# flo-audio/flo

Hardware: AMD Instinct MI355X
Metric: Msamples/s encoded (44.1k stereo, q=high) (higher is better)
Workload: dtype f32

## Files before the change

### diag/lds_model.py

```python
#!/usr/bin/env python3
import argparse
import re
from collections import Counter

import numpy as np

N, HOP, NB = 2048, 1024, 25
SLOT_CAP = 96
ROW = 1024
EDGES = np.array([0, 100, 200, 300, 400, 510, 630, 770, 920, 1080, 1270, 1480, 1720, 2000, 2320, 2700, 3150, 3700,
                  4400, 5300, 6400, 7700, 9500, 12000, 15500, 20500], dtype=np.float32)

R_WIN, R_TW, R_F1, R_F2, R_LANE, R_KEEP, R_DST, R_S10 = 0, 8, 12, 16, 20, 21, 25, 32


def bands(rate):
    res = np.float32(rate) / np.float32(N)
    band = []
    for k in range(HOP):
        f = (np.float32(k) + np.float32(0.5)) * res
        b = NB - 1
        for i in range(1, 26):
            if f < EDGES[i]:
                b = i - 1
# ... 24 lines not shown
    return lane_bnd, lane_slot0, band_slot0, dirty


G128 = [[0, 1, 2, 3, 12, 13, 14, 15] + list(range(20, 28)), [4, 5, 6, 7, 8, 9, 10, 11, 16, 17, 18, 19] + list(range(28, 32))]
G128 = G128 + [[l + 32 for l in g] for g in G128]
G32 = [list(range(0, 32)), list(range(32, 64))]


def contig(n):
    return [list(range(i, i + n)) for i in range(0, 64, n)]


RULES = {
    "ds_read_b32": [(G32, 1, 32)], "ds_write_b32": [(G32, 1, 32)], "ds_write_b16": [(G32, 1, 32)],
    "ds_read_b64": [(G32, 2, 64)], "ds_read_b128": [(G128, 4, 64)],
    "ds_read2_b32": [(G32, 1, 32), (G32, 1, 32)], "ds_write2_b32": [(G32, 1, 32), (G32, 1, 32)],
    "ds_read2_b64": [(contig(16), 2, 32), (contig(16), 2, 32)],
    "ds_write_b64": [(contig(16), 2, 32)], "ds_write_b128": [(contig(8), 4, 32)],
    "ds_write2_b64": [(contig(16), 2, 32), (contig(16), 2, 32)],
}
SKIP_EMPTY = False
GATHER_MASKS = False


def cost(kind, addrs):
    acc = RULES[kind]
    lists = addrs if len(acc) == 2 else [addrs]
    cyc = base = 0
    for (groups, dw, nbank), ad in zip(acc, lists):
        for g in groups:
            per_bank = {}
            for l in g:
                if ad[l] is None:
                    continue
                for i in range(dw):
                    d = ad[l] // 4 + i
                    per_bank.setdefault(d % nbank, set()).add(d)
            if SKIP_EMPTY and not per_bank:
                continue
            cyc += max([len(v) for v in per_bank.values()] or [1])
            base += 1
    return cyc, cyc - base


def lanes(f):
    return [f(l) for l in range(64)]


def sites(rate, layout):
    lane_bnd, lane_slot0, band_slot0, dirty = band_tables(rate)
    row = lambda r, off=0: lanes(lambda l: r * ROW + 16 * l + off)
    uni = lambda a: lanes(lambda l: a)
    one = lambda a: [a] + [None] * 63
    S = []
    S += [("frame", "peek consumed / coef counters", "ds_read_b32", uni(0x8000))] * 2
    S += [("frame", "kRowS10 (uniform)", "ds_read_b128", uni(R_S10 * ROW))] * 2
    if layout == "old":
        S += [("frame", "rcount: kRowLane .z", "ds_read_b32", row(R_LANE, 8))]
    else:
        S += [("frame", "rcount: kRowS10 dword 64 + lane", "ds_read_b32", lanes(lambda l: R_S10 * ROW + 256 + 4 * l))]
    for ph, rr in (("fft pass 1", R_F1), ("fft pass 2", R_F2)):
        S += [(ph, "twiddle rows", "ds_read_b128", row(rr + k)) for k in range(3)]
        S += [(ph, "twiddle row 4 (.xy)", "ds_read_b64", row(rr + 3))]
    X = 0x10000
    for ka in range(8):
        S += [("fft exchange 1", "writes", "ds_write_b128", lanes(lambda l: X + 16 * ((8 * ka + (l & 7)) * 9 + (l >> 3))))]
    for r in range(8):
        S += [("fft exchange 1", "reads", "ds_read_b128", lanes(lambda l: X + 16 * (l * 9 + r)))]
    T = X + 16000
    S += [("masking pass", "ts_ready peek", "ds_read_b32", uni(0x8004))]
    S += [("masking pass", "ts (tl, sf)", "ds_write2_b32", [lanes(lambda l: T + 16 * (l & 31) + 4 * (l >> 5) + o if (l & 31) < 25 else None) for o in (0, 8)])]
    S += [("masking pass", "sfwh", "ds_write_b16", lanes(lambda l: T + 1024 + 2 * l if (l & 31) < 25 else None))]
    S += [("masking pass", "alive", "ds_write_b64", one(T + 1200))]
    S += [("masking pass", "ts_ready", "ds_write_b32", one(0x8004))]
    for kb in range(8):
        S += [("fft exchange 2", "writes", "ds_write_b128", lanes(lambda l: X + 16 * (((l >> 3) + 8 * kb) * 9 + (l & 7))))]
    for r in range(8):
        S += [("fft exchange 2", "reads", "ds_read_b128", lanes(lambda l: X + 16 * (l * 9 + r)))]
    pl = lambda l: 2 * l + 2 * (l >> 3)
    for r in range(8):
        if layout == "old" or r % 2 == 0:
            if layout == "old":
                S += [("post-rotation", "twiddle rows (half rows)", "ds_read_b64", row(R_TW + r // 2, 8 * (r & 1)))]
            else:
                S += [("post-rotation", "twiddle rows", "ds_read_b128", row(R_TW + r // 2))]
        S += [("post-rotation", "transpose writes (2m)", "ds_write_b64", lanes(lambda l: X + 8 * (pl(l) + 144 * r)))]
        S += [("post-rotation", "transpose writes (1023-2m)", "ds_write_b64", lanes(lambda l: X + 8 * (1149 - pl(l) - 144 * r)))]
    for q in range(8):
        S += [("post-rotation", "transpose reads", "ds_read_b128", lanes(lambda l: X + 16 * (9 * l) + 16 * q))]
    S += [("band statistics", "coef_ready", "ds_write_b32", one(0x8008))]
    es = [e for e in range(16) if (dirty >> e) & 1]
    if layout == "old":
        for rr in (R_KEEP, R_DST):
            for g in range(4):
                comp = [e - 4 * g for e in es if 4 * g <= e < 4 * g + 4 and (rr == R_DST or e < 15)]
                i = 0
                while i < len(comp):
                    if i + 1 < len(comp) and comp[i + 1] == comp[i] + 1 and comp[i] % 2 == 1:
                        S += [("band statistics", "keep / dst rows (dword pieces)", "ds_read2_b32", [row(rr + g, 4 * comp[i]), row(rr + g, 4 * comp[i] + 4)])]
                        i += 2
                    elif i + 1 < len(comp) and comp[i + 1] == comp[i] + 1:
                        S += [("band statistics", "keep / dst rows (dword pieces)", "ds_read_b64", row(rr + g, 4 * comp[i]))]
                        i += 2
                    else:
                        S += [("band statistics", "keep / dst rows (dword pieces)", "ds_read_b32", row(rr + g, 4 * comp[i]))]
                        i += 1
    elif layout == "new":
        S += [("band statistics", "keep / dst rows (whole rows)", "ds_read_b128", row(rr + g)) for rr in (R_KEEP, R_DST) for g in range(4)]
    SL = X + 9216
    masks = layout == "masks"
    for e in es:
        def dst(l, e=e, off=0):
            m = lane_bnd[l]
            if (m >> e) & 1:
                return SL + 16 * (lane_slot0[l] + bin(m & ((1 << e) - 1)).count("1")) + off
            return None if masks else SL + 16 * (SLOT_CAP + l)
        if masks and e == 15:
            S += [("band statistics", "slot store (element 15, all lanes)", "ds_write_b128", lanes(dst))]
        elif masks:
            S += [("band statistics", "slot stores (closing lanes)", "ds_write2_b64", [lanes(dst), lanes(lambda l: dst(l, off=8))])]
        else:
            S += [("band statistics", "slot stores", "ds_write_b128", lanes(dst))]
    zero = SLOT_CAP + 64
    for u in range(12):
        def src(l, u=u):
            b = min(l & 31, 24)
            bs0 = band_slot0[b] + (l >> 5)
            bs1 = band_slot0[b + 1] if (l & 31) < 25 else 0
            s = bs0 + 2 * u
            if masks and GATHER_MASKS and not bs0 + 2 * 4 * (u // 4) < bs1:
                return None
            return SL + 16 * (s if s < bs1 else zero)
        S += [("band statistics", "slot gathers", "ds_read_b128", lanes(src))]
    for r in range(8):
        S += [("fold", "window rows", "ds_read_b128", row(R_WIN + r))]
    if layout == "old":
        for k in range(4):
            S += [("fold", "twiddle rows (read2_b64)", "ds_read2_b64", [row(R_TW + k), row(R_TW + k, 8)])]
    else:
        S += [("fold", "twiddle rows", "ds_read_b128", row(R_TW + k)) for k in range(4)]
    return S


def isa_mix(path):
    txt = open(path).read().split("\n")
    start = next(i for i, t in enumerate(txt) if re.match(r"^_ZN3flo20lossy_chain2q_kernelILb0ELj(\d+)ELb0EE.*:", t)
                 and "Lj65535E" not in t)
    body = txt[start:]
    e = next(i for i, t in enumerate(body) if re.match(r"^\.LBB\d+_\d+:.*_clEjS\d_S\d_S\d_S\d_\.exit", t))
    a = max(i for i, t in enumerate(body[:e]) if re.match(r"^\.LBB\d+_\d+:\s+; %\.lr\.ph\d*$", t))
    lab = body[e].split(":")[0]
    c = next(i for i, t in enumerate(body) if i > a and re.search(r"s_cbranch\w*\s+" + re.escape(lab) + r"\b", t))
    b = next(i for i, t in enumerate(body) if i > e and re.match(r"^\.LBB", t))
    mix, cold = Counter(), Counter()
    for i in range(a, b):
        m = re.search(r"\b(ds_[a-z0-9_]+)", body[i])
        if m:
            (cold if c <= i < e else mix)[m.group(1)] += 1
    return mix, cold


def main():
    ap = argparse.ArgumentParser()
    ap.add_argument("--rate", type=int, default=44100)
    ap.add_argument("--layout", default="old", choices=["old", "new", "masks"])
    ap.add_argument("--skip-empty", action="store_true")
    ap.add_argument("--gather-masks", action="store_true")
    ap.add_argument("--isa")
    a = ap.parse_args()
    global SKIP_EMPTY, GATHER_MASKS
    SKIP_EMPTY, GATHER_MASKS = a.skip_empty, a.gather_masks
    S = sites(a.rate, a.layout)
    tab = {}
    tot_c = tot_x = 0
    for ph, site, kind, ad in S:
        c, x = cost(kind, ad)
        k = (ph, site, kind)
        n, cc, xx = tab.get(k, (0, 0, 0))
        tab[k] = (n + 1, cc + c, xx + x)
        tot_c += c
        tot_x += x
    print(f"{'phase':16} {'site':38} {'instruction':14} {'n':>3} {'array':>6} {'conflict':>8}")
    for (ph, site, kind), (n, c, x) in tab.items():
        print(f"{ph:16} {site:38} {kind:14} {n:3d} {c:6d} {x:8d}")
    print(f"{'transform wave, one stereo frame':70} {len(S):3d} {tot_c:6d} {tot_x:8d}")
    if a.isa:
        mix, cold = isa_mix(a.isa)
        model = Counter(kind for _, _, kind, _ in S)
        print("ISA mix (one frame):", dict(sorted(mix.items())), " cold loop (not run at this rate):", dict(cold))
        print("model mix          :", dict(sorted(model.items())))


if __name__ == "__main__":
    main()
```

### flo_amd/csrc/lossy_device.hpp

```cpp
#pragma once
#include <hip/hip_runtime.h>
#include <stdint.h>

#include "pack_rows.h"

namespace flo {


struct LossyDevTables {
    const float4 *pack;
    const float4 *pack_g;
    const float4 *pack_ext;
    const float *ath_db;
    const uint8_t *band;
    const float *band_count;
    const float *s10d;
    const uint32_t *lane_bnd;
    const uint32_t *lane_slot0;
    const uint32_t *band_slot0;
    int max_band_slots;
    uint32_t dirty;
    float smr_thr;
    int q_transparent;
};
// ... 278 lines not shown
    const char *base = reinterpret_cast<const char *>(pcm + s0 * nch + c0);
    const unsigned stride = 4u * (unsigned)nch;
#pragma unroll
    for (int r = 0; r < 8; r++) {
        int eo, oo;
        half_offsets(lane, r, eo, oo);
        const unsigned be = (unsigned)eo * stride, bo = (unsigned)oo * stride;
        if (CH == 2) {
            float2 a = *reinterpret_cast<const float2 *>(base + be);
            float2 b = *reinterpret_cast<const float2 *>(base + bo);
            he[0][r] = a.x;
            he[CH - 1][r] = a.y;
            ho[0][r] = b.x;
            ho[CH - 1][r] = b.y;
        } else {
            he[0][r] = *reinterpret_cast<const float *>(base + be);
            ho[0][r] = *reinterpret_cast<const float *>(base + bo);
        }
    }
}

template <int CH>
__device__ __forceinline__ void fold(const int lane, const float (&ae)[CH][8], const float (&ao)[CH][8], const float (&be)[CH][8],
                                     const float (&bo)[CH][8], float (&zr)[CH][8], float (&zi)[CH][8],
                                     const LossyDevTables &T) {
#pragma unroll
    for (int r = 0; r < 8; r++) {
        const float4 ww = T.pack[(kRowWin + r) * 64 + lane];
        const float wae = ww.x, wao = ww.y, wbe = ww.z, wbo = ww.w;
        const float4 t4 = T.pack[(kRowTw + (r >> 1)) * 64 + lane];
        const float2 w = (r & 1) ? make_float2(t4.z, t4.w) : make_float2(t4.x, t4.y);
#pragma unroll
        for (int c = 0; c < CH; c++) {
            float re, im;
            if (r < 4) {
                re = fmaf(-bo[c][r], wbo, -(be[c][r] * wbe));
                im = fmaf(ao[c][r], wao, -(ae[c][r] * wae));
            } else {
                re = fmaf(-ao[c][r], wao, ae[c][r] * wae);
                im = fmaf(-bo[c][r], wbo, -(be[c][r] * wbe));
            }
            zr[c][r] = fmaf(-im, w.y, -(re * w.x));
            zi[c][r] = fmaf(re, w.y, -(im * w.x));
        }
    }
}

template <int CH>
__device__ __forceinline__ void post_rotate_transpose(const int lane, const float (&zr)[CH][8], const float (&zi)[CH][8],
                                                      float (*coef)[kCoefFloats], float (&c)[CH][16],
                                                      const LossyDevTables &T) {
#pragma unroll
    for (int r = 0; r < 8; r++) {
        const int m = lane + 64 * r;
        const float4 t4 = T.pack[(kRowTw + (r >> 1)) * 64 + lane];
        const float2 w = (r & 1) ? make_float2(t4.z, t4.w) : make_float2(t4.x, t4.y);
        const int k0 = 2 * m, k1 = 1023 - 2 * m;
        const int p0 = k0 + 4 * (k0 >> 5), p1 = k1 + 4 * (k1 >> 5);
#pragma unroll
        for (int ch = 0; ch < CH; ch++) {
            float R = fmaf(-zi[ch][r], w.y, -(zr[ch][r] * w.x));
            float I = fmaf(zi[ch][r], w.x, -(zr[ch][r] * w.y));
            coef[ch][p0] = R;
            coef[ch][p1] = I;
        }
    }
    wave_sync();
#pragma unroll
    for (int ch = 0; ch < CH; ch++) {
        const float4 *p = reinterpret_cast<const float4 *>(&coef[ch][16 * lane + 4 * (lane >> 1)]);
#pragma unroll
        for (int q = 0; q < 4; q++) {
            float4 v = p[q];
            c[ch][4 * q + 0] = v.x;
            c[ch][4 * q + 1] = v.y;
            c[ch][4 * q + 2] = v.z;
            c[ch][4 * q + 3] = v.w;
        }
    }
    wave_sync();
}

typedef float v2f __attribute__((ext_vector_type(2)));
__device__ __forceinline__ v2f fma2(v2f a, v2f b, v2f c) { return __builtin_elementwise_fma(a, b, c); }
__device__ __forceinline__ v2f fma2_na_hi_nc(v2f a, v2f w, v2f c) {
    v2f r;
    asm("v_pk_fma_f32 %0, %1, %2, %3 op_sel:[0,1,0] op_sel_hi:[1,1,1] neg_lo:[1,0,1] neg_hi:[1,0,1]" : "=v"(r) : "v"(a), "v"(w), "v"(c));
    return r;
}
__device__ __forceinline__ v2f fma2_a_hi_c(v2f a, v2f w, v2f c) {
    v2f r;
    asm("v_pk_fma_f32 %0, %1, %2, %3 op_sel:[0,1,0] op_sel_hi:[1,1,1]" : "=v"(r) : "v"(a), "v"(w), "v"(c));
    return r;
}
__device__ __forceinline__ v2f mul2_hi(v2f a, v2f w) {
    v2f r;
    asm("v_pk_mul_f32 %0, %1, %2 op_sel:[0,1] op_sel_hi:[1,1]" : "=v"(r) : "v"(a), "v"(w));
    return r;
}
__device__ __forceinline__ v2f fma2_a_hi_nc(v2f a, v2f w, v2f c) {
    v2f r;
    asm("v_pk_fma_f32 %0, %1, %2, %3 op_sel:[0,1,0] op_sel_hi:[1,1,1] neg_lo:[0,0,1] neg_hi:[0,0,1]" : "=v"(r) : "v"(a), "v"(w), "v"(c));
    return r;
}
__device__ __forceinline__ v2f splat2(float x) { return (v2f){x, x}; }

constexpr int kXch4 = 64 * kXchStride;
constexpr int kCoef2 = 1024 + 2 * 64;

__device__ __forceinline__ void dft8_2(v2f *xr, v2f *xi) {
    const v2f s = splat2(0.70710678118654752440f);
    v2f a0r = xr[0] + xr[4], a0i = xi[0] + xi[4];
    v2f a1r = xr[0] - xr[4], a1i = xi[0] - xi[4];
    v2f a2r = xr[2] + xr[6], a2i = xi[2] + xi[6];
    v2f a3r = xr[2] - xr[6], a3i = xi[2] - xi[6];
    v2f a4r = xr[1] + xr[5], a4i = xi[1] + xi[5];
    v2f a5r = xr[1] - xr[5], a5i = xi[1] - xi[5];
    v2f a6r = xr[3] + xr[7], a6i = xi[3] + xi[7];
    v2f a7r = xr[3] - xr[7], a7i = xi[3] - xi[7];
    v2f b0r = a0r + a2r, b0i = a0i + a2i;
    v2f b2r = a0r - a2r, b2i = a0i - a2i;
    v2f b1r = a1r + a3i, b1i = a1i - a3r;
    v2f b3r = a1r - a3i, b3i = a1i + a3r;
    v2f c0r = a4r + a6r, c0i = a4i + a6i;
    v2f c2r = a4r - a6r, c2i = a4i - a6i;
    v2f c1r = a5r + a7i, c1i = a5i - a7r;
    v2f c3r = a5r - a7i, c3i = a5i + a7r;
    const v2f e1r = c1r + c1i, e1i = c1i - c1r;
    const v2f e3r = c3i - c3r, e3i = c3r + c3i;
    xr[0] = b0r + c0r; xi[0] = b0i + c0i;
    xr[4] = b0r - c0r; xi[4] = b0i - c0i;
    xr[1] = fma2(e1r, s, b1r); xi[1] = fma2(e1i, s, b1i);
    xr[5] = fma2(-e1r, s, b1r); xi[5] = fma2(-e1i, s, b1i);
    xr[2] = b2r + c2i; xi[2] = b2i - c2r;
    xr[6] = b2r - c2i; xi[6] = b2i + c2r;
    xr[3] = fma2(e3r, s, b3r); xi[3] = fma2(-e3i, s, b3i);
    xr[7] = fma2(-e3r, s, b3r); xi[7] = fma2(e3i, s, b3i);
}

__device__ __forceinline__ void cmul_2(v2f &xr, v2f &xi, float wr, float wi) {
    const v2f WR = splat2(wr), WI = splat2(wi);
    v2f r = fma2(xr, WR, -(xi * WI));
    v2f i = fma2(xr, WI, xi * WR);
    xr = r;
    xi = i;
}
__device__ __forceinline__ void cmul_2_pair(v2f &xr, v2f &xi, v2f w) {
    const v2f WR = splat2(w.x);
    v2f r = fma2(xr, WR, -mul2_hi(xi, w));
    v2f i = fma2_a_hi_c(xr, w, xi * WR);
    xr = r;
    xi = i;
}

struct NoShadow { __device__ __forceinline__ void operator()() const {} };
template <typename F = NoShadow>
__device__ __forceinline__ void fft512_2(const int lane, v2f (&zr)[8], v2f (&zi)[8], float4 *x4, const LossyDevTables &T, F &&shadow = F()) {
    dft8_2(zr, zi);
#pragma unroll
    for (int kk = 0; kk < 4; kk++) {
        const float4 w = T.pack[(kRowF1 + kk) * 64 + lane];
        cmul_2(zr[2 * kk + 1], zi[2 * kk + 1], w.x, w.y);
        if (kk < 3) cmul_2_pair(zr[2 * kk + 2], zi[2 * kk + 2], (v2f){w.z, w.w});
    }
    {
        const int nb = lane >> 3, nc = lane & 7;
#pragma unroll
        for (int ka = 0; ka < 8; ka++) x4[(8 * ka + nc) * kXchStride + nb] = make_float4(zr[ka].x, zr[ka].y, zi[ka].x, zi[ka].y);
        wave_sync();
#pragma unroll
        for (int r = 0; r < 8; r++) {
            const float4 v = x4[lane * kXchStride + r];
            zr[r] = (v2f){v.x, v.y};
            zi[r] = (v2f){v.z, v.w};
        }
        shadow();
        wave_sync();
    }
    dft8_2(zr, zi);
#pragma unroll
    for (int kk = 0; kk < 4; kk++) {
        const float4 w = T.pack[(kRowF2 + kk) * 64 + lane];
        cmul_2(zr[2 * kk + 1], zi[2 * kk + 1], w.x, w.y);
        if (kk < 3) cmul_2_pair(zr[2 * kk + 2], zi[2 * kk + 2], (v2f){w.z, w.w});
    }
    {
        const int ka = lane >> 3, nc = lane & 7;
#pragma unroll
        for (int kb = 0; kb < 8; kb++) x4[(ka + 8 * kb) * kXchStride + nc] = make_float4(zr[kb].x, zr[kb].y, zi[kb].x, zi[kb].y);
        wave_sync();
#pragma unroll
        for (int r = 0; r < 8; r++) {
            const float4 v = x4[lane * kXchStride + r];
            zr[r] = (v2f){v.x, v.y};
            zi[r] = (v2f){v.z, v.w};
        }
        wave_sync();
    }
    dft8_2(zr, zi);
}

__device__ __forceinline__ void load_half_fast_2(const int lane, const float *__restrict__ pcm, long long s0, v2f (&he)[8], v2f (&ho)[8]) {
    const char *base0 = reinterpret_cast<const char *>(pcm + s0 * 2);
    const char *base1 = base0 + 4096;
    const unsigned va = 16u * (unsigned)lane, vb = 16u * (unsigned)(63 - lane);
#pragma unroll
    for (int r = 0; r < 8; r++) {
        const int rr = r & 3;
        const char *pe = (r < 4 ? base1 : base0) + va + 1024 * rr;
        const char *po = (r < 4 ? base0 : base1) + vb + (3080 - 1024 * rr);
        const float2 a = *reinterpret_cast<const float2 *>(pe);
        const float2 b = *reinterpret_cast<const float2 *>(po);
        he[r] = (v2f){a.x, a.y};
        ho[r] = (v2f){b.x, b.y};
    }
}

__device__ __forceinline__ void fold_2(const int lane, const v2f (&ae)[8], const v2f (&ao)[8], const v2f (&be)[8], const v2f (&bo)[8],
                                       v2f (&zr)[8], v2f (&zi)[8], const LossyDevTables &T) {
    float4 t4;
#pragma unroll
    for (int r = 0; r < 8; r++) {
        const float4 ww = T.pack[(kRowWin + r) * 64 + lane];
        const v2f wae = splat2(ww.x), wao = splat2(ww.y), wbe = splat2(ww.z);
        const v2f whi = {ww.z, ww.w};
        if (!(r & 1)) t4 = pack_row(&T.pack[(kRowTw + (r >> 1)) * 64 + lane]);
        const v2f wx = splat2((r & 1) ? t4.z : t4.x);
        const v2f thi = {t4.z, t4.w};
        v2f re, im;
        if (r < 4) {
            re = fma2_na_hi_nc(bo[r], whi, be[r] * wbe);
            im = fma2(ao[r], wao, -(ae[r] * wae));
        } else {
            re = fma2(-ao[r], wao, ae[r] * wae);
            im = fma2_na_hi_nc(bo[r], whi, be[r] * wbe);
        }
        if (r & 1) {
            zr[r] = fma2_na_hi_nc(im, thi, re * wx);
            zi[r] = fma2_a_hi_nc(re, thi, im * wx);
        } else {
            const v2f wy = splat2(t4.y);
            zr[r] = fma2(-im, wy, -(re * wx));
            zi[r] = fma2(re, wy, -(im * wx));
        }
    }
}

__device__ __forceinline__ void post_rotate_transpose_2(const int lane, const v2f (&zr)[8], const v2f (&zi)[8], float2 *c2,
                                                        v2f (&c)[16], const LossyDevTables &T) {
    const int pl = 2 * lane + 2 * (lane >> 3);
    float2 *const w0 = c2 + pl;
    float2 *const w1 = c2 + (1149 - 7 * 144) - pl;
    float4 t4;
#pragma unroll
    for (int r = 0; r < 8; r++) {
        if (!(r & 1)) t4 = pack_row(&T.pack[(kRowTw + (r >> 1)) * 64 + lane]);
        const v2f wx = splat2((r & 1) ? t4.z : t4.x);
        v2f R, I;
        if (r & 1) {
            const v2f thi = {t4.z, t4.w};
            R = fma2_na_hi_nc(zi[r], thi, zr[r] * wx);
            I = fma2(zi[r], wx, -mul2_hi(zr[r], thi));
        } else {
            const v2f wy = splat2(t4.y);
            R = fma2(-zi[r], wy, -(zr[r] * wx));
            I = fma2(zi[r], wx, -(zr[r] * wy));
        }
        w0[144 * r] = make_float2(R.x, R.y);
        w1[144 * (7 - r)] = make_float2(I.x, I.y);
    }
    wave_sync();
    const float4 *p = reinterpret_cast<const float4 *>(&c2[18 * lane]);
#pragma unroll
    for (int q = 0; q < 8; q++) {
        const float4 v = p[q];
        c[2 * q] = (v2f){v.x, v.y};
        c[2 * q + 1] = (v2f){v.z, v.w};
    }
    wave_sync();
}

struct LaneConst {
    float rcount;
};

__device__ __forceinline__ void load_lane_const(const int lane, LaneConst &L, const LossyDevTables &T) {
    L.rcount = T.pack[kRowLane * 64 + lane].z;
}

constexpr int kZeroSlot = kSlotCap + 64;

template <int CH>
__device__ __forceinline__ void band_stats(const int lane, const float (&c)[CH][16], float2 (*slots)[kSlotCap + 64 + 1],
                                           const LossyDevTables &T, float (&energy)[CH], float (&bmax)[CH]) {
    float kp[16];
    uint32_t dv[16], so[12];
#pragma unroll
    for (int g = 0; g < 4; g++) {
        const float4 keep = T.pack[(kRowKeep + g) * 64 + lane];
        const float4 dsto = T.pack[(kRowDst + g) * 64 + lane];
        kp[4 * g + 0] = keep.x, kp[4 * g + 1] = keep.y, kp[4 * g + 2] = keep.z, kp[4 * g + 3] = keep.w;
        dv[4 * g + 0] = __float_as_uint(dsto.x), dv[4 * g + 1] = __float_as_uint(dsto.y);
        dv[4 * g + 2] = __float_as_uint(dsto.z), dv[4 * g + 3] = __float_as_uint(dsto.w);
    }
#pragma unroll
    for (int g = 0; g < 3; g++) {
        const float4 lst = T.pack[(kRowLst + g) * 64 + lane];
        so[4 * g + 0] = __float_as_uint(lst.x), so[4 * g + 1] = __float_as_uint(lst.y);
        so[4 * g + 2] = __float_as_uint(lst.z), so[4 * g + 3] = __float_as_uint(lst.w);
    }
    __builtin_amdgcn_sched_barrier(0);
    float acc[CH], mx[CH];
#pragma unroll
    for (int ch = 0; ch < CH; ch++) {
        acc[ch] = 0.f;
        mx[ch] = 0.f;
    }
#pragma unroll
    for (int e = 0; e < 16; e++) {
#pragma unroll
        for (int ch = 0; ch < CH; ch++) {
            acc[ch] = fmaf(c[ch][e], c[ch][e], acc[ch]);
            mx[ch] = max_abs_raw(mx[ch], c[ch][e]);
            *reinterpret_cast<float2 *>(reinterpret_cast<char *>(slots[ch]) + dv[e]) = make_float2(acc[ch], mx[ch]);
            acc[ch] *= kp[e];
            mx[ch] *= kp[e];
        }
    }
    wave_sync();
    float2 v[CH][12];
#pragma unroll
    for (int u = 0; u < 12; u++)
#pragma unroll
        for (int ch = 0; ch < CH; ch++)
            v[ch][u] = *reinterpret_cast<const float2 *>(reinterpret_cast<const char *>(slots[ch]) + so[u]);
    __builtin_amdgcn_sched_barrier(0);
#pragma unroll
    for (int ch = 0; ch < CH; ch++) {
        energy[ch] = 0.f;
        bmax[ch] = 0.f;
    }
#pragma unroll
    for (int u = 0; u < 12; u++)
#pragma unroll
        for (int ch = 0; ch < CH; ch++) {
            energy[ch] += v[ch][u].x;
            bmax[ch] = max_raw(bmax[ch], v[ch][u].y);
        }
    const int groups = (T.max_band_slots + 7) >> 3;
    for (int g = 3; g < groups; g++) {
// ... 916 lines not shown
```

### flo_amd/csrc/lossy_kernels.hip

```cpp
#include <assert.h>
#include <stdlib.h>

#include <mutex>
#include <set>
#include <type_traits>
#include <utility>

#include "chain2q_roles.hpp"
#include "crc_device.hpp"
#include "lossy_device.hpp"
#include "lossy_kernels.hpp"
#include "../../include/flo_synth.h"

#ifndef FLO_SKIP
#define FLO_SKIP 0
#endif
#define FLO_KEEP(x) asm volatile("" ::"v"(x))
#ifdef FLO_STAMPS
#define STAMP(i)                                                                                  \
    do {                                                                                          \
        __builtin_amdgcn_sched_barrier(0);                                                        \
        unsigned long long t_;                                                                    \
        asm volatile("s_memtime %0\n\ts_waitcnt lgkmcnt(0)" : "=s"(t_)::"memory");              \
        __builtin_amdgcn_sched_barrier(0);                                                        \
// ... 534 lines not shown
                    uint32_t t = sparse_item_pack(ln, xd[ch], f_a + pos + 4u, tab_a);
#ifdef FLO_STAMPS
                    if (t == kSparseFallback) st_sum[6] += 1;
#endif
                    if (t == kSparseFallback) t = sparse_block_pack(ln, xd[ch], f_a + pos + 4u, tab_a);
#else
                    uint32_t t = 3u + ((xd[ch][0] | xd[ch][3]) & 1u);
                    FLO_KEEP(xd[ch][1]); FLO_KEEP(xd[ch][2]); FLO_KEEP(xd[ch][4]); FLO_KEEP(xd[ch][5]); FLO_KEEP(xd[ch][6]); FLO_KEEP(xd[ch][7]);
#endif
                    if (t == kSparseFallback) {
                        uint32_t *scr = reinterpret_cast<uint32_t *>(stage + 2560);
#pragma unroll
                        for (int k = 0; k < 8; k++) scr[64 * k + ln] = xd[ch][k];
                        wave_sync();
                        const uint4 x0 = reinterpret_cast<const uint4 *>(scr)[2 * ln], x1 = reinterpret_cast<const uint4 *>(scr)[2 * ln + 1];
                        wave_sync();
                        const uint32_t xs[8] = {x0.x, x0.y, x0.z, x0.w, x1.x, x1.y, x1.z, x1.w};
                        int q[1][16];
                        uint32_t hi[8];
#pragma unroll
                        for (int k = 0; k < 8; k++) {
                            hi[k] = xs[k] >> 16;
                            q[0][2 * k] = (int)xs[k];
                            q[0][2 * k + 1] = (int)hi[k];
                        }
                        SparsePlan P[1];
                        sparse_plan_m(ln, nonzero_mask16_packed(xs, hi), P[0]);
                        uint8_t *const dsts[1] = {f + pos + 4};
                        const uint32_t trash[1] = {(uint32_t)((stage + kFrameCap + 64 + 2 * ln) - dsts[0])};
                        sparse_emit_n<1>(ln, q, P, dsts, trash);
                        t = P[0].total;
                    }
                    tot[ch] = t;
                    pos += 4u + t;
                    if (ch == 0) take_next();
                    STAMP(2 + ch);
                }
                const uint32_t flen = pos, blob_len = flen - 10;
                {
                    const uint32_t i = (uint32_t)ln;
                    const uint32_t w0 = 0x000400FDu, w1 = blob_len << 16, w2 = (blob_len >> 16) | 0x02000000u;
                    uint32_t wv4 = i < 4u ? w0 : (i < 8u ? w1 : w2);
                    wv4 = i < 12u ? wv4 : (i < 16u ? tot[0] : tot[1]);
                    const uint32_t off = i < 12u ? i : (i < 16u ? 112u - 12u + i : 116u - 16u + tot[0] + i);
                    const uint32_t bv = wv4 >> (8u * (i & 3u));
                    if (i < 20u) lds_st8<0>(f + off, bv);
                    if (ln == 0) A.frame_size[frame0 + h] = flen;
                }
                wave_sync();
                take_next();
                const uint32_t haveb = pend + flen;
                const uint32_t n16 = haveb >> 4;
                const uint4 *src = reinterpret_cast<const uint4 *>(stage);
                uint4 *dst = reinterpret_cast<uint4 *>(gout + written);
                for (uint32_t i = ln; i < n16; i += 64) dst[i] = src[i];
                pend = haveb & 15u;
                tailb = (ln < (int)pend) ? stage[(n16 << 4) + ln] : 0u;
                written += (unsigned long long)n16 << 4;
                wave_sync();
                STAMP(4);
#ifdef FLO_STAMPS
                {
                    const unsigned long long busy = st_last - st_frame0;
                    if (busy > 12000) { st_sum[9] += busy; st_sum[10] += 1; }
                    if (busy > 20000) { st_sum[11] += busy; st_sum[12] += 1; }
                }
#endif
            }
            if (lane < (int)pend) gout[written + lane] = (uint8_t)tailb;
            if (lane == 0) A.clip_bytes[clip] = written + pend;
            done_clip = clip;
            done_bytes = written + pend;
            STAMPS_RECORD(1);
            fbase += hops;
        }
    }

    LossyDevTables T = A.T;
    T.pack = reinterpret_cast<const float4 *>(lds_raw);
    uint32_t so_pre[12], slot_first;
    band_stats_2_prepare(lane, cs.slot, A.T.pack, so_pre, slot_first);
    unsigned long long close[16];
    band_stats_2_masks<DIRTY>(masks, close);
    for (;;) {
        wait_counter(&cs.clip_seq, ++seq);
        const unsigned clip = (unsigned)__builtin_amdgcn_readfirstlane((int)cs.clip_cur);
        if (clip >= (unsigned)A.n_clips) return;
        const unsigned hops = A.clip_hops[clip];
        const unsigned long long frame0 = A.clip_frame0[clip];
        const float *pcm = A.pcm + A.clip_off[clip];

        float prev = 0.f;
        v2f ae[8], ao[8], be[8], bo[8];
#pragma unroll
        for (int r = 0; r < 8; r++) ae[r] = ao[r] = splat2(0.f);
        if (!COEFFS) load_half_fast_2(lane_id_opaque(), pcm, 0, be, bo);
        STAMPS_BEGIN();
        v2f zr[8], zi[8];
        if (!COEFFS) fold_2(lane_id_opaque(), ae, ao, be, bo, zr, zi, T);
        float pend_e = 0.f, pend_m = 0.f;
        auto mask_publish = [&](const int ln, const uint32_t gp, const unsigned hp, const float energy1, const float bmax1,
                                const float rcount, const float4 sd0, const float4 sd1) __attribute__((always_inline)) {
            const int bnd = ln & 31, up = ln >> 5;
#if (FLO_SKIP & 16) == 0
            const float bm = bmax1;
            const float sfv1 = bm > 1e-10f ? __fdiv_rn(30000.0f, bm) : 1.0f;
            const uint32_t sfw1 = sf_word(sfv1);
            const float a = spread_threshold_2r(ln, energy1, rcount, sd0, sd1, T);
            const float sl = max_raw(a, prev * 0.7f);
            prev = sl;
            const float tl1 = masking_amplitude(sl, T.smr_thr);
#else
            const float bm = bmax1, tl1 = energy1 * 1e-3f + rcount + sd0.x + sd1.y, sfv1 = bm * 100.f + 1.f;
            const uint32_t sfw1 = __float_as_uint(tl1) >> 16;
#endif
            const unsigned long long al = __ballot(bnd < 25 && bm > tl1);
            if (bnd < 25) {
                typedef __attribute__((address_space(3))) float lds_f32;
                const uint32_t ts_s = (uint32_t)__builtin_amdgcn_readfirstlane((int)(uint32_t)(uintptr_t)cs.ts[gp & 1u]);
                lds_f32 *tp = reinterpret_cast<lds_f32 *>((uintptr_t)(ts_s + 16u * (uint32_t)bnd + 4u * (uint32_t)up));
                tp[0] = tl1;
                tp[2] = sfv1;
                cs.sfwh[gp & 1u][up][bnd] = (uint16_t)sfw1;
            }
            if (ln == 0) {
                cs.alive[gp & 1u][0] = (uint32_t)al;
                cs.alive[gp & 1u][1] = (uint32_t)(al >> 32);
            }
            if (DBG && A.dbg_sfw && bnd < 25) A.dbg_sfw[((frame0 + hp) * 2 + up) * 25 + bnd] = (unsigned short)sfw1;
            set_counter(&cs.ts_ready, gp + 1);
        };
        auto frame_body = [&](const unsigned h, v2f (&ne)[8], v2f (&no)[8], v2f (&fe)[8], v2f (&fo)[8]) __attribute__((always_inline)) {
            const int ln = lane_id_opaque();
            const uint32_t g = fbase + h;
            FLO_MARK("frame_begin");
            const uint32_t consumed_early = peek_counter(&cs.consumed);
            const float4 sd0 = T.pack[kRowS10 * 64], sd1 = T.pack[kRowS10 * 64 + 1];
            const float rcount = reinterpret_cast<const float *>(T.pack + kRowS10 * 64)[64 + ln];
            v2f c[16];
            if (COEFFS) {
#pragma unroll
                for (int q = 0; q < 4; q++) {
                    const float4 v0 = reinterpret_cast<const float4 *>(A.in_coeffs + ((frame0 + h) * 2 + 0) * 1024 + 16 * ln)[q];
                    const float4 v1 = reinterpret_cast<const float4 *>(A.in_coeffs + ((frame0 + h) * 2 + 1) * 1024 + 16 * ln)[q];
                    c[4 * q] = (v2f){v0.x, v1.x}; c[4 * q + 1] = (v2f){v0.y, v1.y};
                    c[4 * q + 2] = (v2f){v0.z, v1.z}; c[4 * q + 3] = (v2f){v0.w, v1.w};
                }
                if ((uint32_t)__builtin_amdgcn_readfirstlane((int)consumed_early) < g) wait_counter(&cs.consumed, g);
                float4 *p = reinterpret_cast<float4 *>(&cs.u.coef2[18 * ln]);
#pragma unroll
                for (int q = 0; q < 8; q++) p[q] = make_float4(c[2 * q].x, c[2 * q].y, c[2 * q + 1].x, c[2 * q + 1].y);
                wave_sync();
            } else {
                load_half_fast_2(ln, pcm, (long long)(h + 1) * 1024, ne, no);
                FLO_MARK("prefetch_done");
                STAMP(1);
                if ((uint32_t)__builtin_amdgcn_readfirstlane((int)consumed_early) < g) wait_counter(&cs.consumed, g);
                STAMP(7);
#if (FLO_SKIP & 8) == 0
                fft512_2(ln, zr, zi, cs.u.xch4, T, [&]() __attribute__((always_inline)) {
                    if (h > 0) mask_publish(ln, g - 1u, h - 1u, pend_e, pend_m, rcount, sd0, sd1);
                });
#else
                if (h > 0) mask_publish(ln, g - 1u, h - 1u, pend_e, pend_m, rcount, sd0, sd1);
#endif
                FLO_MARK("fft_done");
                STAMP(2);
#if (FLO_SKIP & 4) == 0
                post_rotate_transpose_2(ln, zr, zi, cs.u.coef2, c, T);
#else
#pragma unroll
                for (int e = 0; e < 8; e++) { c[2 * e] = zr[e]; c[2 * e + 1] = zi[e]; }
#endif
                FLO_MARK("postrot_done");
                STAMP(3);
                if (DBG && A.dbg_coeffs) {
#pragma unroll
                    for (int ch = 0; ch < 2; ch++) {
                        float *d = A.dbg_coeffs + ((frame0 + h) * 2 + ch) * 1024 + 16 * ln;
#pragma unroll
                        for (int e = 0; e < 16; e++) d[e] = ch ? c[e].y : c[e].x;
                    }
                }
            }
            set_counter(&cs.coef_ready, g + 1);
            float energy1, bmax1;
#if (FLO_SKIP & 1) == 0
            band_stats_2<DIRTY, true, true>(ln, c, cs.slot, T, energy1, bmax1, so_pre, close, slot_first);
#else
            energy1 = c[0].x + c[5].y;
            bmax1 = c[1].x + c[7].y;
#endif
            FLO_MARK("bandstats_done");
            STAMP(4);
            if (COEFFS) {
                mask_publish(ln, g, h, energy1, bmax1, rcount, sd0, sd1);
            } else {
                pend_e = energy1, pend_m = bmax1;
#if (FLO_SKIP & 128) == 0
                fold_2(ln, fe, fo, ne, no, zr, zi, T);
#else
#pragma unroll
                for (int r = 0; r < 8; r++) { zr[r] = fe[r] + ne[r]; zi[r] = fo[r] - no[r]; }
#endif
            }
            FLO_MARK("frame_end");
            STAMP(5);
        };
        for (unsigned h = 0; h < hops; h += 2) {
            frame_body(h, ae, ao, be, bo);
            if (h + 1 < hops) frame_body(h + 1, be, bo, ae, ao);
        }
        if (!COEFFS && hops) {
            const int ln = lane_id_opaque();
            const float4 sd0 = T.pack[kRowS10 * 64], sd1 = T.pack[kRowS10 * 64 + 1];
            mask_publish(ln, fbase + hops - 1u, hops - 1u, pend_e, pend_m, reinterpret_cast<const float *>(T.pack + kRowS10 * 64)[64 + ln], sd0, sd1);
        }
        STAMPS_RECORD(0);
        fbase += hops;
    }
}

template <int CH, int STEP, bool EXACT>
__global__ __launch_bounds__(64) void lossy_frame_kernel(LossyArgs A) {
    constexpr int PASS = STEP & ~kStreamStep;
    constexpr bool STREAM = (STEP & kStreamStep) != 0;
    __shared__ WaveLds<CH> lds;
    __shared__ __attribute__((aligned(16))) uint8_t stage[kFrameCap + 64 + 256];
    const int lane = lane_id();
    const unsigned long long gframe = blockIdx.x;
    if (gframe >= A.total_frames) return;
    int lo = 0, hi = A.n_clips - 1;
    while (lo < hi) {
        int mid = (lo + hi + 1) >> 1;
        if (A.clip_frame0[mid] <= gframe) lo = mid; else hi = mid - 1;
    }
    const unsigned clip = (unsigned)lo;
    const unsigned h = (unsigned)(gframe - A.clip_frame0[clip]);
    const float *pcm = A.pcm + A.clip_off[clip];
    const long long n_sf = (long long)A.clip_nsf[clip];

    LaneConst L;
    load_lane_const(lane, L, A.T);
    if (lane < CH) lds.slots[lane][kZeroSlot] = make_float2(0.f, 0.f);
    float c[CH][16];
    if (A.in_coeffs) {
        load_coeffs<CH>(lane, c, A, gframe, 0);
    } else {
        float ae[CH][8], ao[CH][8], be[CH][8], bo[CH][8];
        load_half<CH>(lane, pcm, n_sf, A.nch, 0, (long long)(h + STREAM) * 1024 - 1024, ae, ao);
        load_half<CH>(lane, pcm, n_sf, A.nch, 0, (long long)(h + STREAM) * 1024, be, bo);
        mdct_frame<CH>(lane, ae, ao, be, bo, lds, A.T, c);
    }
    FrameState<CH> st;
    int q[CH][16];
    uint32_t sfw[CH];
    SparsePlan P[CH];
    if (PASS == 1) {
#pragma unroll
        for (int ch = 0; ch < CH; ch++) st.prev[ch] = 0.f;
        analyse_frame<CH, true, EXACT>(lane, c, lds, L, A, A.T, 0, st, gframe, q, sfw, P);
        if (lane < 25) {
#pragma unroll
            for (int ch = 0; ch < CH; ch++) mark_inf_level(A, clip, (unsigned)ch, (unsigned)lane, h, A.a_t[(gframe * A.nch + ch) * 32 + lane]);
        }
        return;
    }
    store_coeffs_dbg<CH>(lane, c, A, gframe, 0);
#pragma unroll
    for (int ch = 0; ch < CH; ch++) st.prev[ch] = lane < 25 ? A.s_prev[(gframe * A.nch + ch) * 32 + lane] : 0.f;
    analyse_frame<CH, false, EXACT>(lane, c, lds, L, A, A.T, 0, st, gframe, q, sfw, P);
    uint32_t tot[2];
    tot[0] = P[0].total;
    tot[1] = P[CH - 1].total;
    const uint32_t flen = emit_frame<CH>(lane, stage, CH, 0, tot, sfw, P, q);
    wave_sync();
    if (lane == 0) A.frame_size[gframe] = flen;
    const uint32_t n16 = (flen + 15) >> 4;
    const uint4 *src = reinterpret_cast<const uint4 *>(stage);
    uint4 *dst = reinterpret_cast<uint4 *>(A.slots + gframe * (unsigned long long)A.slot_bytes);
    for (uint32_t i = lane; i < n16; i += 64) dst[i] = src[i];
}

constexpr int kScanBlock = 64;
struct QuantOnlyLds {
    float4 ts[32];
    uint32_t qh[2][512];
};
template <int STEP, bool FROMCOEF = false>
__global__ __launch_bounds__(64) void lossy_frame2x_kernel(LossyArgs A) {
    constexpr int PASS = STEP & ~kStreamStep;
    constexpr bool STREAM = (STEP & kStreamStep) != 0;
    constexpr bool kSmall = PASS == 2 && FROMCOEF;
    __shared__ typename std::conditional<kSmall, QuantOnlyLds, StereoLds>::type lds;
    __shared__ __attribute__((aligned(16))) uint8_t stage[PASS == 2 ? kFrameCap + 64 + 256 : 16];
// ... 902 lines not shown
```

### profiles/phase_table.py

```python
#!/usr/bin/env python3
import collections
import re
import sys


def classify(op):
    if op.startswith("v_"):
        return "valu"
    if op.startswith("ds_"):
        return "lds"
    if op.startswith("s_waitcnt"):
        return "wait"
    if op.startswith(("global_", "buffer_", "flat_", "scratch_")):
        return "vmem"
    if op.startswith("s_load") or op.startswith("s_buffer_load"):
        return "smem"
    if op.startswith("s_"):
        return "salu"
    return None


def main():
    path = sys.argv[1]
    want = sys.argv[2] if len(sys.argv) > 2 else "lossy_chain2q_kernelILb0ELj48574ELb0EE"
    lines = open(path).read().split("\n")
    start = next(i for i, l in enumerate(lines) if l.startswith("_Z") and want in l and ":" in l.split(";")[0])
    end = next(i for i in range(start, len(lines)) if ".size" in lines[i] and want in lines[i])
    phases = collections.OrderedDict()
    cur = "pre (clip set-up, packer wave)"
    order = []
    for l in lines[start:end]:
        s = l.strip()
        m = re.match(r"; MARK (\w+)", s)
        if m:
            cur = m.group(1)
            continue
        if not s or s.startswith((";", ".", "//")) or s.endswith(":"):
            continue
        op = s.split()[0]
        k = classify(op)
        if k is None:
            continue
        phases.setdefault(cur, collections.Counter())[k] += 1
        if cur not in order:
            order.append(cur)
    names = {"frame_begin": "prefetch (16 loads), masking rows", "prefetch_done": "fft512 x2 + masking pass (prev. frame)",
             "fft_done": "post-rotation + transpose", "postrot_done": "band_stats_2",
             "bandstats_done": "fold of the next frame (a)", "frame_end": "fold of the next frame (b), loop"}
    print(f"{'phase':32s} {'VALU':>6s} {'SALU':>6s} {'LDS':>5s} {'VMEM':>5s} {'wait':>5s}   (per stereo frame, mean of the two unrolled bodies)")
    tot = collections.Counter()
    for ph in order:
        c = phases[ph]
        nm = names.get(ph, ph)
        div = 1 if ph.startswith("pre (") else 2
        row = {k: c[k] / div for k in ("valu", "salu", "lds", "vmem", "wait")}
        if not ph.startswith("pre ("):
            for k, v in row.items():
                tot[k] += v
        print(f"{nm:32s} {row['valu']:6.0f} {row['salu']:6.0f} {row['lds']:5.0f} {row['vmem']:5.0f} {row['wait']:5.0f}")
    print(f"{'transform wave, per frame':32s} {tot['valu']:6.0f} {tot['salu']:6.0f} {tot['lds']:5.0f} {tot['vmem']:5.0f} {tot['wait']:5.0f}")


if __name__ == "__main__":
    main()
```

Before: 697,500.

## Carry fold overlap half across frames and keep twiddles in registers

The MDCT fold now computes the windowed contribution of each half-frame once and carries it in registers to the next frame, instead of keeping both previous and next half buffers and swapping them via a two-body unrolled loop. Twiddle rows are loaded once per kernel into registers and reused by both the fold and the post-rotation, removing per-frame LDS/pack reads of those rows. The frame loop is no longer unrolled by two, which shrinks code but may lose some scheduling freedom and raises register pressure with the persistent twiddle and carry arrays.

```diff
diff --git a/diag/lds_model.py b/diag/lds_model.py
--- a/diag/lds_model.py
+++ b/diag/lds_model.py
@@ -130,7 +130,7 @@
         if layout == "old" or r % 2 == 0:
             if layout == "old":
                 S += [("post-rotation", "twiddle rows (half rows)", "ds_read_b64", row(R_TW + r // 2, 8 * (r & 1)))]
-            else:
+            elif layout != "carry":
                 S += [("post-rotation", "twiddle rows", "ds_read_b128", row(R_TW + r // 2))]
         S += [("post-rotation", "transpose writes (2m)", "ds_write_b64", lanes(lambda l: X + 8 * (pl(l) + 144 * r)))]
         S += [("post-rotation", "transpose writes (1023-2m)", "ds_write_b64", lanes(lambda l: X + 8 * (1149 - pl(l) - 144 * r)))]
@@ -156,7 +156,7 @@
     elif layout == "new":
         S += [("band statistics", "keep / dst rows (whole rows)", "ds_read_b128", row(rr + g)) for rr in (R_KEEP, R_DST) for g in range(4)]
     SL = X + 9216
-    masks = layout == "masks"
+    masks = layout in ("masks", "carry")
     for e in es:
         def dst(l, e=e, off=0):
             m = lane_bnd[l]
@@ -185,7 +185,7 @@
     if layout == "old":
         for k in range(4):
             S += [("fold", "twiddle rows (read2_b64)", "ds_read2_b64", [row(R_TW + k), row(R_TW + k, 8)])]
-    else:
+    elif layout != "carry":
         S += [("fold", "twiddle rows", "ds_read_b128", row(R_TW + k)) for k in range(4)]
     return S
 
@@ -211,7 +211,7 @@
 def main():
     ap = argparse.ArgumentParser()
     ap.add_argument("--rate", type=int, default=44100)
-    ap.add_argument("--layout", default="old", choices=["old", "new", "masks"])
+    ap.add_argument("--layout", default="old", choices=["old", "new", "masks", "carry"])
     ap.add_argument("--skip-empty", action="store_true")
     ap.add_argument("--gather-masks", action="store_true")
     ap.add_argument("--isa")
diff --git a/flo_amd/csrc/lossy_device.hpp b/flo_amd/csrc/lossy_device.hpp
--- a/flo_amd/csrc/lossy_device.hpp
+++ b/flo_amd/csrc/lossy_device.hpp
@@ -384,6 +384,12 @@
 }
 
 typedef float v2f __attribute__((ext_vector_type(2)));
+typedef float v4f __attribute__((ext_vector_type(4)));
+__device__ __forceinline__ v4f pack_row_v(const float4 *p) {
+    v4f v = *reinterpret_cast<const v4f *>(p);
+    asm("" : "+v"(v));
+    return v;
+}
 __device__ __forceinline__ v2f fma2(v2f a, v2f b, v2f c) { return __builtin_elementwise_fma(a, b, c); }
 __device__ __forceinline__ v2f fma2_na_hi_nc(v2f a, v2f w, v2f c) {
     v2f r;
@@ -403,6 +409,16 @@
 __device__ __forceinline__ v2f fma2_a_hi_nc(v2f a, v2f w, v2f c) {
     v2f r;
     asm("v_pk_fma_f32 %0, %1, %2, %3 op_sel:[0,1,0] op_sel_hi:[1,1,1] neg_lo:[0,0,1] neg_hi:[0,0,1]" : "=v"(r) : "v"(a), "v"(w), "v"(c));
+    return r;
+}
+__device__ __forceinline__ v2f mul2_lo(v2f a, v2f w) {
+    v2f r;
+    asm("v_pk_mul_f32 %0, %1, %2 op_sel:[0,0] op_sel_hi:[1,0]" : "=v"(r) : "v"(a), "v"(w));
+    return r;
+}
+__device__ __forceinline__ v2f fma2_a_lo_nc(v2f a, v2f w, v2f c) {
+    v2f r;
+    asm("v_pk_fma_f32 %0, %1, %2, %3 op_sel:[0,0,0] op_sel_hi:[1,0,1] neg_lo:[0,0,1] neg_hi:[0,0,1]" : "=v"(r) : "v"(a), "v"(w), "v"(c));
     return r;
 }
 __device__ __forceinline__ v2f splat2(float x) { return (v2f){x, x}; }
@@ -568,6 +584,54 @@
             R = fma2(-zi[r], wy, -(zr[r] * wx));
             I = fma2(zi[r], wx, -(zr[r] * wy));
         }
+        w0[144 * r] = make_float2(R.x, R.y);
+        w1[144 * (7 - r)] = make_float2(I.x, I.y);
+    }
+    wave_sync();
+    const float4 *p = reinterpret_cast<const float4 *>(&c2[18 * lane]);
+#pragma unroll
+    for (int q = 0; q < 8; q++) {
+        const float4 v = p[q];
+        c[2 * q] = (v2f){v.x, v.y};
+        c[2 * q + 1] = (v2f){v.z, v.w};
+    }
+    wave_sync();
+}
+
+__device__ __forceinline__ v2f fold_a_part(const int r, const v2f he, const v2f ho, const float4 ww) {
+    const v2f wae = splat2(ww.x), wao = splat2(ww.y);
+    return r < 4 ? fma2(ho, wao, -(he * wae)) : fma2(-ho, wao, he * wae);
+}
+__device__ __forceinline__ void fold_carry_init_2(const int lane, v2f (&acar)[8], const LossyDevTables &T) {
+#pragma unroll
+    for (int r = 0; r < 8; r++) acar[r] = fold_a_part(r, splat2(0.f), splat2(0.f), T.pack[(kRowWin + r) * 64 + lane]);
+}
+__device__ __forceinline__ void fold_carry_2(const int lane, const v2f (&ne)[8], const v2f (&no)[8], v2f (&acar)[8],
+                                             const v4f (&tw)[4], v2f (&zr)[8], v2f (&zi)[8], const LossyDevTables &T) {
+#pragma unroll
+    for (int r = 0; r < 8; r++) {
+        const float4 ww = T.pack[(kRowWin + r) * 64 + lane];
+        const v2f wbe = splat2(ww.z);
+        const v2f whi = {ww.z, ww.w};
+        const v2f t2 = (r & 1) ? tw[r >> 1].zw : tw[r >> 1].xy;
+        const v2f bp = fma2_na_hi_nc(no[r], whi, ne[r] * wbe);
+        const v2f re = r < 4 ? bp : acar[r], im = r < 4 ? acar[r] : bp;
+        zr[r] = fma2_na_hi_nc(im, t2, mul2_lo(re, t2));
+        zi[r] = fma2_a_hi_nc(re, t2, mul2_lo(im, t2));
+        acar[r] = fold_a_part(r, ne[r], no[r], ww);
+    }
+}
+
+__device__ __forceinline__ void post_rotate_transpose_2_tw(const int lane, const v2f (&zr)[8], const v2f (&zi)[8], float2 *c2,
+                                                           v2f (&c)[16], const v4f (&tw)[4]) {
+    const int pl = 2 * lane + 2 * (lane >> 3);
+    float2 *const w0 = c2 + pl;
+    float2 *const w1 = c2 + (1149 - 7 * 144) - pl;
+#pragma unroll
+    for (int r = 0; r < 8; r++) {
+        const v2f t2 = (r & 1) ? tw[r >> 1].zw : tw[r >> 1].xy;
+        const v2f R = fma2_na_hi_nc(zi[r], t2, mul2_lo(zr[r], t2));
+        const v2f I = fma2_a_lo_nc(zi[r], t2, mul2_hi(zr[r], t2));
         w0[144 * r] = make_float2(R.x, R.y);
         w1[144 * (7 - r)] = make_float2(I.x, I.y);
     }
diff --git a/flo_amd/csrc/lossy_kernels.hip b/flo_amd/csrc/lossy_kernels.hip
--- a/flo_amd/csrc/lossy_kernels.hip
+++ b/flo_amd/csrc/lossy_kernels.hip
@@ -640,6 +640,11 @@
     band_stats_2_prepare(lane, cs.slot, A.T.pack, so_pre, slot_first);
     unsigned long long close[16];
     band_stats_2_masks<DIRTY>(masks, close);
+    v4f tw[4];
+    if (!COEFFS) {
+#pragma unroll
+        for (int k = 0; k < 4; k++) tw[k] = pack_row_v(&T.pack[(kRowTw + k) * 64 + lane]);
+    }
     for (;;) {
         wait_counter(&cs.clip_seq, ++seq);
         const unsigned clip = (unsigned)__builtin_amdgcn_readfirstlane((int)cs.clip_cur);
@@ -649,13 +654,14 @@
         const float *pcm = A.pcm + A.clip_off[clip];
 
         float prev = 0.f;
-        v2f ae[8], ao[8], be[8], bo[8];
-#pragma unroll
-        for (int r = 0; r < 8; r++) ae[r] = ao[r] = splat2(0.f);
-        if (!COEFFS) load_half_fast_2(lane_id_opaque(), pcm, 0, be, bo);
+        v2f ne[8], no[8], acar[8];
+        if (!COEFFS) {
+            fold_carry_init_2(lane_id_opaque(), acar, T);
+            load_half_fast_2(lane_id_opaque(), pcm, 0, ne, no);
+        }
         STAMPS_BEGIN();
         v2f zr[8], zi[8];
-        if (!COEFFS) fold_2(lane_id_opaque(), ae, ao, be, bo, zr, zi, T);
+        if (!COEFFS) fold_carry_2(lane_id_opaque(), ne, no, acar, tw, zr, zi, T);
         float pend_e = 0.f, pend_m = 0.f;
         auto mask_publish = [&](const int ln, const uint32_t gp, const unsigned hp, const float energy1, const float bmax1,
                                 const float rcount, const float4 sd0, const float4 sd1) __attribute__((always_inline)) {
@@ -688,7 +694,7 @@
             if (DBG && A.dbg_sfw && bnd < 25) A.dbg_sfw[((frame0 + hp) * 2 + up) * 25 + bnd] = (unsigned short)sfw1;
             set_counter(&cs.ts_ready, gp + 1);
         };
-        auto frame_body = [&](const unsigned h, v2f (&ne)[8], v2f (&no)[8], v2f (&fe)[8], v2f (&fo)[8]) __attribute__((always_inline)) {
+        auto frame_body = [&](const unsigned h) __attribute__((always_inline)) {
             const int ln = lane_id_opaque();
             const uint32_t g = fbase + h;
             FLO_MARK("frame_begin");
@@ -725,7 +731,7 @@
                 FLO_MARK("fft_done");
                 STAMP(2);
 #if (FLO_SKIP & 4) == 0
-                post_rotate_transpose_2(ln, zr, zi, cs.u.coef2, c, T);
+                post_rotate_transpose_2_tw(ln, zr, zi, cs.u.coef2, c, tw);
 #else
 #pragma unroll
                 for (int e = 0; e < 8; e++) { c[2 * e] = zr[e]; c[2 * e + 1] = zi[e]; }
@@ -756,19 +762,16 @@
             } else {
                 pend_e = energy1, pend_m = bmax1;
 #if (FLO_SKIP & 128) == 0
-                fold_2(ln, fe, fo, ne, no, zr, zi, T);
+                fold_carry_2(ln, ne, no, acar, tw, zr, zi, T);
 #else
 #pragma unroll
-                for (int r = 0; r < 8; r++) { zr[r] = fe[r] + ne[r]; zi[r] = fo[r] - no[r]; }
+                for (int r = 0; r < 8; r++) { zr[r] = acar[r] + ne[r]; zi[r] = acar[r] - no[r]; }
 #endif
             }
             FLO_MARK("frame_end");
             STAMP(5);
         };
-        for (unsigned h = 0; h < hops; h += 2) {
-            frame_body(h, ae, ao, be, bo);
-            if (h + 1 < hops) frame_body(h + 1, be, bo, ae, ao);
-        }
+        for (unsigned h = 0; h < hops; h++) frame_body(h);
         if (!COEFFS && hops) {
             const int ln = lane_id_opaque();
             const float4 sd0 = T.pack[kRowS10 * 64], sd1 = T.pack[kRowS10 * 64 + 1];
diff --git a/profiles/phase_table.py b/profiles/phase_table.py
--- a/profiles/phase_table.py
+++ b/profiles/phase_table.py
@@ -29,7 +29,11 @@
     phases = collections.OrderedDict()
     cur = "pre (clip set-up, packer wave)"
     order = []
-    for l in lines[start:end]:
+    bodies = max(1, sum(1 for l in lines[start:end] if l.strip().startswith("; MARK frame_begin")))
+    last_end = max((i for i in range(start, end) if lines[i].strip().startswith("; MARK frame_end")), default=end)
+    for i, l in enumerate(lines[start:end], start):
+        if i == last_end + 1:
+            cur = "post (behind the last frame_end)"
         s = l.strip()
         m = re.match(r"; MARK (\w+)", s)
         if m:
@@ -47,14 +51,15 @@
     names = {"frame_begin": "prefetch (16 loads), masking rows", "prefetch_done": "fft512 x2 + masking pass (prev. frame)",
              "fft_done": "post-rotation + transpose", "postrot_done": "band_stats_2",
              "bandstats_done": "fold of the next frame (a)", "frame_end": "fold of the next frame (b), loop"}
-    print(f"{'phase':32s} {'VALU':>6s} {'SALU':>6s} {'LDS':>5s} {'VMEM':>5s} {'wait':>5s}   (per stereo frame, mean of the two unrolled bodies)")
+    print(f"{'phase':32s} {'VALU':>6s} {'SALU':>6s} {'LDS':>5s} {'VMEM':>5s} {'wait':>5s}   (per stereo frame, {bodies} frame bod{'y' if bodies == 1 else 'ies'})")
     tot = collections.Counter()
     for ph in order:
         c = phases[ph]
         nm = names.get(ph, ph)
-        div = 1 if ph.startswith("pre (") else 2
+        once = ph.startswith(("pre (", "post ("))
+        div = 1 if once else bodies
         row = {k: c[k] / div for k in ("valu", "salu", "lds", "vmem", "wait")}
-        if not ph.startswith("pre ("):
+        if not once:
             for k, v in row.items():
                 tot[k] += v
         print(f"{nm:32s} {row['valu']:6.0f} {row['salu']:6.0f} {row['lds']:5.0f} {row['vmem']:5.0f} {row['wait']:5.0f}")
```

Result: faster. 706,100, median of 6 (+1.2%).
